# firedrakeproject/fiat

Hardware: AMD Instinct MI355X
Metric: element tabulations/sec (basis+grad, fp64) for batched P3 tet (higher is better)
Workload: dtype f64; 1 GPU; Lagrange degree 3 tetrahedron, order 1, 23 points/request, batch 100000 per GPU; requests_per_gpu=100000, points_per_request=23, order=1, points=random per request, world_size=1, launch=single process, clock_ramp_steps=224

## Files before the change

fiat_amd/csrc/api.hip:

```cpp
#include <hip/hip_runtime.h>

#include <algorithm>
#include <cmath>
#include <cstdarg>
#include <cstdio>
#include <cstring>
#include <cstdlib>
#include <mutex>
#include <string>
#include <thread>
#include <numeric>
#include <vector>

#include "../../include/fiat_amd.h"
#include "aux_kernels.hpp"
#include "plan.hpp"
#include "simplex_kernel.hpp"
#include "simplex_fixed.hpp"
#include "simplex_stream.hpp"
#include "simplex_pair.hpp"
#include "coop_kernel.hpp"
#include "shared_points.hpp"
#include "quadrature.hpp"
#include "simplex_small.hpp"
// ... 1688 lines not shown
                        !(order == 0 && vec3_rows && npts >= 17 && npts <= 24) &&
                        !(verts && order != 1 && (hi14 || hi_more)) &&
                        !(want_mix && wg_mix_takes(k)))
                        continue;
                    wg_g = npts > 64 ? 1 : std::min(12, 128 / npts);
                    wg_ctw = std::max(4, (wg_g * npts + 15) / 16);
                    if (want_mix) {
                        wg_ctw = fxwg::mix_ct(k.sd, k.n, wg_ctw);
                        wg_odd = ((long long)rows * npts) % 2 || ((long long)(rows - 16 * ((rows + 15) / 16 - 1)) * npts) % 2;
                        wg_mix1 = wg_ctw > 0 && fxwg::has_mix_instance(k.sd, k.n, wg_ctw, wg_odd) && wg_mix_takes(k);
                    }
                    if (!wg_mix1) {
                        if (verts && order >= 1 && npts <= 48 && !(ctx->policy & FX_POLICY_WG_SMALL) && !(hi14 && order == 2)) continue;
                        wg_odd = !even;
                        wg_ctw = std::max(4, (wg_g * npts + 15) / 16);
                        if (wg_ctw == 7) wg_ctw = 8;
                        if (wg_ctw == 5) {
                            const long long one = (long long)((RT + 3) / 4) * 5, two = (long long)((RT + 1) / 2) * 3;
                            if (two < one || wg_g > 1) wg_ctw = 6;
                        }
                        if (npts > 64 && (wg_g * npts + 15) / 16 <= 6 && !(ctx->policy & FX_POLICY_WG_SMALL) &&
                            !((e->nexp + 3) / 4 >= 14 || (k.sd == 2 && k.n == 6 && order == 2) || wg_ctw == 5))
                            continue;
                        if (!fxwg::has_instance(k.sd, k.n, wg_ctw, wg_odd)) continue;
                    }
                    if (!wg_mix1 && npts > 48 && npts <= 64 && even && !(ctx->policy & FX_POLICY_WG_SMALL) && !(k.sd == 3 && k.n >= 5)) {
                        bool whole = false;
                        for (const StackedShape& o : kStackedShapes)
                            whole = whole || (o.sd == k.sd && o.n == k.n && o.rtc == 0 && o.g == 1 && o.ct == 4);
                        if (whole) continue;
                    }
                    if (nreq + 3LL * ctx->num_cu > 0x7fffffffLL) continue;
                } else if (chunked) {
                    if (npts < 13 || nreq * (long long)((npts + 16 * k.ct - 1) / (16 * k.ct)) > 0x7fffffffLL) continue;
                    if ((k.rtc == -1 || k.rtc == -4) && k.sd == 3 && (k.n == 6 || k.n == 5)) {
                        const long long t2 = 2LL * ((npts + 31) / 32), t3 = 3LL * ((npts + 47) / 48);
                        if ((k.ct == 2) != (t2 < t3)) continue;
                    }
                    if (inmix) {
                        const bool nomix = (ctx->policy & FX_POLICY_NO_STACKED_MIX) != 0;
                        if (nomix || !verts || order != (k.rtc == -4 ? 1 : 2) || npts <= 16 * k.ct) continue;
                        if (k.rtc == -4 && wg_mix_takes(k)) continue;
                        if (npts <= 64 && even && R <= 224 && !(order == 2 && k.sd == 2 && k.n == 6)) {
                            bool whole = false;
                            for (const StackedShape& o : kStackedShapes)
                                whole = whole || (o.sd == k.sd && o.n == k.n && o.rtc == 0 && o.g == 1 && o.ct == 4);
                            if (whole) continue;
                        }
                    }
                } else {
                    const bool odd_twin = (k.sd == 3 && k.n == 4 && k.ct == 3 && k.g == 2) || (k.sd == 3 && k.n == 2 && k.ct == 3 && (k.g == 2 || k.g == 4)) ||
                                          (k.sd == 3 && k.n == 3 && k.ct == 3 && k.g == 2) || (k.sd == 2 && k.n == 5 && k.ct == 2 && k.g == 1);
                    if (!even && !odd_twin) continue;
                    if (npts > 16 * k.ct / k.g || tighter_instance(k) || !fills_tiles(k)) continue;
                }
                bool ok = false;
                if (e->sd == 3 && e->n == 6) ok = table_matches<3, 6>(e->prog);
                if (e->sd == 3 && e->n == 5) ok = table_matches<3, 5>(e->prog);
                if (e->sd == 3 && e->n == 4) ok = table_matches<3, 4>(e->prog);
                if (e->sd == 3 && e->n == 3) ok = table_matches<3, 3>(e->prog);
                if (e->sd == 2 && e->n == 6) ok = table_matches<2, 6>(e->prog);
                if (e->sd == 2 && e->n == 5) ok = table_matches<2, 5>(e->prog);
                if (e->sd == 3 && e->n == 2) ok = table_matches<3, 2>(e->prog);
                if (e->sd == 2 && e->n == 4) ok = table_matches<2, 4>(e->prog);
                if (e->sd == 2 && e->n == 3) ok = table_matches<2, 3>(e->prog);
                if (e->sd == 3 && e->n == 7) ok = table_matches<3, 7>(e->prog);
                if (e->sd == 2 && e->n == 7) ok = table_matches<2, 7>(e->prog);
                if (e->sd == 2 && e->n == 8) ok = table_matches<2, 8>(e->prog);
                if (!ok) continue;
                int rc = ensure_stacked(ctx, const_cast<fx_element*>(e), order);
                if (rc != FX_OK) return rc;
                if (e->stack_state[order] != 1) continue;
                fxk::StackedArgs<0>& ka = L.khead;
                memset(&ka, 0, sizeof ka);
                L.fcoef.resize(e->prog.steps.size() * 3);
                for (size_t q = 0; q < e->prog.steps.size(); ++q) {
                    L.fcoef[3 * q + 0] = e->prog.steps[q].A;
                    L.fcoef[3 * q + 1] = e->prog.steps[q].B;
                    L.fcoef[3 * q + 2] = e->prog.steps[q].C;
                }
                ka.pts = pts;
                ka.verts = verts;
                ka.out = out;
                const bool dofmajor = inmix || wg_mix1;
                ka.afrag = pio ? e->d_astack_dmp[order] : dofmajor ? e->d_astack_dm[order] : e->d_astack[order];
                if (!ka.afrag) continue;
                if (pio) {
                    for (int q = 0; q < 9; ++q) ka.G[q] = 0.5 * e->A0[q];
                    ka.piola = mapping;
                }
                if (dofmajor && !invert_small(e->sd, e->A0, ka.A0inv)) continue;
                ka.phi0 = e->prog.phi0;
                memcpy(ka.A0, e->A0, sizeof ka.A0);
                memcpy(ka.b0, e->b0, sizeof ka.b0);
                ka.nreq = nreq;
                ka.npts = npts;
                ka.R = (int)R;
                ka.RT = RT;
                ka.debug = a.debug;
                ka.lim_pts = (long long)nreq * npts * e->sd;
                ka.lim_verts = verts ? (long long)nreq * (e->sd + 1) * e->sd : 0;
                ka.lim_out = (long long)nreq * R * npts;
                const int TRk = fxk::stacked_tile_rows(e->sd, pio ? 1 : 0);
                ka.lim_afrag = (dofmajor ? ((long long)((rows + TRk - 1) / TRk) * ntab + 1) : (long long)(RT + 1)) * ((e->nexp + 3) / 4) * 64;
                const bool mixr = pio || k.rtc == -3 || k.rtc == -4 || k.rtc == -5 || (k.rtc == -2 && (mix_odd || mixr1(k.sd, k.n, k.ct, k.g) || (k.sd == 3 && k.n == 6 && k.ct == 3)));
                const int slots = fxk::stacked_mix_slots(e->sd, dofmajor ? ntab : 0, mixr);
                L.klds_bytes = (fxk::WQ_CTL_DOUBLES + STACKED_NW * (fxk::stacked_image_doubles(k.ct, (e->nexp + 3) / 4, slots) + (mixr ? fxk::STACKED_KBUF : 0))) * 8;
                if (wgk) {
                    L.klds_bytes = fxwg::lds_bytes(k.sd, k.n, wg_ctw);
                    L.wg_ct = wg_ctw;
                    L.wg_mix = wg_mix1 ? 1 : 0;
                    ka.gslab = wg_g;
                }
                if (L.klds_bytes > ctx->lds_per_cu) continue;
                const long long groups = wgk ? ((nreq + wg_g - 1) / wg_g) * STACKED_NW : chunked ? nreq * ((npts + 16 * k.ct - 1) / (16 * k.ct)) : (nreq + k.g - 1) / k.g;
                const int wgs = wgk ? fxwg::workgroups_per_cu(k.sd, k.n, wg_ctw, wg_odd, wg_mix1 ? 1 : 0, RT) : 1;
                L.kgrid = (int)std::max<long long>(1, std::min<long long>((groups + STACKED_NW - 1) / STACKED_NW, (long long)ctx->num_cu * wgs));
                L.ncu = ctx->num_cu;
                L.trash = ctx->d_trash;
                L.ctx = ctx;
                L.kmix_order = order;
                L.kodd = wgk ? wg_odd : ((k.rtc == 0 && !even) || mix_odd);
                L.kpiola = pio ? mapping : 0;
                if (pio) L.fused_mapping = true;
                L.stacked_id = (int)i;
                L.small_id = -1;
                if (fixed_yields) L.fixed_id = -1;
                break;
            }
        }
    }
    int per_cu = std::max(1, std::min(16, ctx->lds_per_cu / std::max(1, L.lds_bytes)));
    long long want = (long long)ctx->num_cu * per_cu * 4;
    L.grid = (int)std::max<long long>(1, std::min<long long>(a.nitems, want));
    return FX_OK;
}

int run_tabulate(fx_ctx* ctx, const fx_element* e, int order, const Launch& L, hipStream_t s) {
    if (L.args.nitems == 0 || L.args.npts == 0) return FX_OK;
    if (L.fixed_id >= 0) return run_fixed(L, s);
    if (L.stacked_id >= 0) return run_stacked(L, s);
    if (L.coop_id >= 0) return run_coop(L, s);
    if (L.small_id >= 0) return run_small(order, L, s);
    switch (e->sd) {
        case 1: return launch_sd<1>(order, L, s);
        case 2: return launch_sd<2>(order, L, s);
        case 3: return launch_sd<3>(order, L, s);
    }
    return fail(FX_EINVAL, "Invalid number of spatial dimensions");
}

}

namespace {
template <int SD, int ORDER, bool PIOLA, int EL>
bool launch_shared_reg_sliced(int units, const fxk::SharedArgs& sa_in, int ncu, hipStream_t s) {
    constexpr int NTAB = fxk::NTab<SD, ORDER>::value;
    constexpr int PER = EL * NTAB * (PIOLA ? SD : 1);
    constexpr int NPMAX = PER >= 80 ? 1 : PER >= 40 ? 2 : PER >= 27 ? 3 : 4;
    const int need = (units + 255) / 256;
    const int np = std::min(need, NPMAX);
    const int slices = (need + np - 1) / np;
    fxk::SharedArgs sa = sa_in;
    const long long want = 4LL * ncu;
    sa.rb = (int)std::max<long long>(1, std::min<long long>(fxk::SHARED_RB, sa.nreq * slices / want));
    const long long blocks = (sa.nreq + sa.rb - 1) / sa.rb;
    const dim3 g((unsigned)std::max<long long>(1, std::min<long long>(blocks, std::max<long long>(1, 8LL * ncu / slices))), (unsigned)slices);
    switch (np) {
        case 1: hipLaunchKernelGGL((fxk::shared_points_reg_kernel<SD, ORDER, 1, PIOLA, EL>), g, dim3(256), 0, s, sa); return true;
        case 2: if constexpr (NPMAX >= 2) { hipLaunchKernelGGL((fxk::shared_points_reg_kernel<SD, ORDER, 2, PIOLA, EL>), g, dim3(256), 0, s, sa); return true; } break;
        case 3: if constexpr (NPMAX >= 3) { hipLaunchKernelGGL((fxk::shared_points_reg_kernel<SD, ORDER, 3, PIOLA, EL>), g, dim3(256), 0, s, sa); return true; } break;
        case 4: if constexpr (NPMAX >= 4) { hipLaunchKernelGGL((fxk::shared_points_reg_kernel<SD, ORDER, 4, PIOLA, EL>), g, dim3(256), 0, s, sa); return true; } break;
    }
    return false;
}

#ifndef FX_SHARED_FLAT_MAX
#define FX_SHARED_FLAT_MAX 12
#endif
static inline bool noflat_shared(unsigned policy) { return (policy & FX_POLICY_NO_SHARED_REG) != 0 && (policy & FX_POLICY_NO_SHARED_WAVE) != 0; }

template <int SD>
int launch_shared(int order, const fxk::SharedArgs& sa, int ncu, hipStream_t s, unsigned policy) {
    const int table = sa.rows * sa.npts;
    const int grid = (int)std::max<long long>(1, std::min<long long>((sa.nreq + fxk::SHARED_RB - 1) / fxk::SHARED_RB, (long long)ncu * 8));
    {
        const long long total = (long long)fx::binom(SD + order, SD) * table;
        if (!noflat_shared(policy) && (total <= FX_SHARED_FLAT_MAX || ((table & 1) && total <= 32)) && (sa.kind == 0 || sa.vdim == SD)) {
            const long long teams = (sa.nreq + 63) / 64;
            const int fgrid = (int)std::max<long long>(1, std::min<long long>((teams + 3) / 4, (long long)grid));
            switch (order) {
                case 0: hipLaunchKernelGGL((fxk::shared_points_flat_kernel<SD, 0>), dim3(fgrid), dim3(256), 0, s, sa); break;
                case 1: hipLaunchKernelGGL((fxk::shared_points_flat_kernel<SD, 1>), dim3(fgrid), dim3(256), 0, s, sa); break;
                default: hipLaunchKernelGGL((fxk::shared_points_flat_kernel<SD, 2>), dim3(fgrid), dim3(256), 0, s, sa); break;
            }
            HIP_TRY(hipGetLastError());
            return FX_OK;
        }
    }
    const bool nowave = (policy & FX_POLICY_NO_SHARED_WAVE) != 0;
    if (!nowave && sa.kind == 0 && order == 1 && (table & 1) == 0) {
        const int npairs = (1 + SD) * table / 2;
        const int ns = (npairs + 63) / 64;
        const int nwr = ns <= 8 ? 1 : ns <= 16 ? 2 : 4;
        const long long teams = (sa.nreq + 63) / 64;
        const int wgrid = (int)std::max<long long>(1, std::min<long long>((teams * nwr + 3) / 4, (long long)grid));
        bool ok = ns <= 32;
        if (ok) hipLaunchKernelGGL((fxk::shared_points_wave_kernel<SD, 8>), dim3(wgrid), dim3(256), 0, s, sa, nwr);
        if (ok) {
            HIP_TRY(hipGetLastError());
            return FX_OK;
        }
    }
    const bool noreg = (policy & FX_POLICY_NO_SHARED_REG) != 0;
    if (!noreg && (sa.kind == 0 || sa.vdim == SD)) {
        const bool piola = sa.kind != 0;
        bool ok = false;
        constexpr bool PIO_EVEN = SD >= 2, PIO_ODD = SD == 3;
        if (table & 1) {
            if (!piola) {
                if (order == 0) ok = launch_shared_reg_sliced<SD, 0, false, 1>(table, sa, ncu, s);
                if (order == 1) ok = launch_shared_reg_sliced<SD, 1, false, 1>(table, sa, ncu, s);
                if (order == 2) ok = launch_shared_reg_sliced<SD, 2, false, 1>(table, sa, ncu, s);
            } else if constexpr (PIO_ODD) {
                if (order == 0) ok = launch_shared_reg_sliced<SD, 0, true, 1>(table, sa, ncu, s);
                if (order == 1) ok = launch_shared_reg_sliced<SD, 1, true, 1>(table, sa, ncu, s);
                if (order == 2) ok = launch_shared_reg_sliced<SD, 2, true, 1>(table, sa, ncu, s);
            }
        } else {
            if (!piola) {
                if (order == 0) ok = launch_shared_reg_sliced<SD, 0, false, 2>(table / 2, sa, ncu, s);
                if (order == 1) ok = launch_shared_reg_sliced<SD, 1, false, 2>(table / 2, sa, ncu, s);
                if (order == 2) ok = launch_shared_reg_sliced<SD, 2, false, 2>(table / 2, sa, ncu, s);
            } else if constexpr (PIO_EVEN) {
                if (order == 0) ok = launch_shared_reg_sliced<SD, 0, true, 2>(table / 2, sa, ncu, s);
                if (order == 1) ok = launch_shared_reg_sliced<SD, 1, true, 2>(table / 2, sa, ncu, s);
                if (order == 2) ok = launch_shared_reg_sliced<SD, 2, true, 2>(table / 2, sa, ncu, s);
            }
        }
        if (ok) {
            HIP_TRY(hipGetLastError());
            return FX_OK;
        }
    }
    const int rgrid = (int)std::max<long long>(1, std::min<long long>(sa.nreq, (long long)ncu * 8));
    switch (order) {
        case 0: hipLaunchKernelGGL((fxk::shared_points_kernel<SD, 0>), dim3(rgrid), dim3(256), 0, s, sa); break;
        case 1: hipLaunchKernelGGL((fxk::shared_points_kernel<SD, 1>), dim3(rgrid), dim3(256), 0, s, sa); break;
        default: hipLaunchKernelGGL((fxk::shared_points_kernel<SD, 2>), dim3(rgrid), dim3(256), 0, s, sa); break;
    }
    HIP_TRY(hipGetLastError());
    return FX_OK;
}
}

namespace {
template <int N, int NN, int ORDER>
void launch_prism_small(const fxk::PrismArgs& a, int grid, size_t lds, hipStream_t s) {
    auto kern = fxk::prism_small_kernel<N, NN, ORDER, 4>;
    if (lds > 48 * 1024) (void)hipFuncSetAttribute(reinterpret_cast<const void*>(kern), hipFuncAttributeMaxDynamicSharedMemorySize, (int)lds);
    hipLaunchKernelGGL(kern, dim3(grid), dim3(256), lds, s, a);
}
template <int N, int NN>
bool launch_prism_small_order(int order, const fxk::PrismArgs& a, int grid, size_t lds, hipStream_t s) {
    if (order == 0) launch_prism_small<N, NN, 0>(a, grid, lds, s);
    else if (order == 1) launch_prism_small<N, NN, 1>(a, grid, lds, s);
    else if (order == 2 && N <= 2 && NN <= 3) {
        if constexpr (N <= 2 && NN <= 3) launch_prism_small<N, NN, 2>(a, grid, lds, s);
    } else return false;
    return true;
}
template <int N>
bool launch_prism_small_nn(int nn, int order, const fxk::PrismArgs& a, int grid, size_t lds, hipStream_t s) {
    switch (nn) {
        case 1: return launch_prism_small_order<N, 1>(order, a, grid, lds, s);
        case 2: return launch_prism_small_order<N, 2>(order, a, grid, lds, s);
        case 3: return launch_prism_small_order<N, 3>(order, a, grid, lds, s);
        case 4: return launch_prism_small_order<N, 4>(order, a, grid, lds, s);
    }
    return false;
}
}

namespace {
template <int NF, int NN, int ORDER>
static void launch_tensor_small(bool grid_mode, const fxk::TensorArgs& a, int P, int img_doubles, int grid, size_t lds, hipStream_t s) {
    if (grid_mode) {
        auto kern = fxk::tensor_small_kernel<NF, NN, ORDER, true>;
        if (lds > 48 * 1024) (void)hipFuncSetAttribute(reinterpret_cast<const void*>(kern), hipFuncAttributeMaxDynamicSharedMemorySize, (int)lds);
        hipLaunchKernelGGL(kern, dim3(grid), dim3(256), lds, s, a, P, img_doubles);
    } else {
        auto kern = fxk::tensor_small_kernel<NF, NN, ORDER, false>;
        if (lds > 48 * 1024) (void)hipFuncSetAttribute(reinterpret_cast<const void*>(kern), hipFuncAttributeMaxDynamicSharedMemorySize, (int)lds);
        hipLaunchKernelGGL(kern, dim3(grid), dim3(256), lds, s, a, P, img_doubles);
    }
}

static bool try_tensor_small(fx_ctx* ctx, bool grid_mode, const fxk::TensorArgs& a, hipStream_t s) {
    if ((ctx->policy & FX_POLICY_NO_SMALL) != 0 || a.nf < 2 || a.npts > 64) return false;
    const int nn = a.L[0].nn;
    for (int f = 1; f < a.nf; ++f)
        if (a.L[f].nn != nn) return false;
    long long ndof = 1;
    for (int f = 0; f < a.nf; ++f) ndof *= nn;
    const long long total = (long long)a.ntab * ndof * a.npts;
    constexpr long long IMG_BYTES = 16 * 1024;
    if (total * 8 > IMG_BYTES) return false;
    const int P = (int)std::max<long long>(1, std::min<long long>(64 / a.npts, IMG_BYTES / (total * 8)));
    const int img_doubles = (int)((P * total + 1) & ~1LL);
    const size_t lds = (size_t)img_doubles * 8 * 4;
    const long long items = (a.nreq + P - 1) / P;
    const int per_cu = (int)std::max<size_t>(1, std::min<size_t>(4, (size_t)ctx->lds_per_cu / std::max<size_t>(lds, 1)));
    const int grid = (int)std::max<long long>(1, std::min<long long>((items + 3) / 4, (long long)ctx->num_cu * per_cu * 2));
    const int key = a.nf * 100 + nn * 10 + a.order;
    switch (key) {
        case 220: launch_tensor_small<2, 2, 0>(grid_mode, a, P, img_doubles, grid, lds, s); return true;
        case 221: launch_tensor_small<2, 2, 1>(grid_mode, a, P, img_doubles, grid, lds, s); return true;
        case 222: launch_tensor_small<2, 2, 2>(grid_mode, a, P, img_doubles, grid, lds, s); return true;
        case 230: launch_tensor_small<2, 3, 0>(grid_mode, a, P, img_doubles, grid, lds, s); return true;
        case 231: launch_tensor_small<2, 3, 1>(grid_mode, a, P, img_doubles, grid, lds, s); return true;
        case 232: launch_tensor_small<2, 3, 2>(grid_mode, a, P, img_doubles, grid, lds, s); return true;
        case 240: launch_tensor_small<2, 4, 0>(grid_mode, a, P, img_doubles, grid, lds, s); return true;
        case 241: launch_tensor_small<2, 4, 1>(grid_mode, a, P, img_doubles, grid, lds, s); return true;
        case 242: launch_tensor_small<2, 4, 2>(grid_mode, a, P, img_doubles, grid, lds, s); return true;
        case 250: launch_tensor_small<2, 5, 0>(grid_mode, a, P, img_doubles, grid, lds, s); return true;
        case 251: launch_tensor_small<2, 5, 1>(grid_mode, a, P, img_doubles, grid, lds, s); return true;
        case 320: launch_tensor_small<3, 2, 0>(grid_mode, a, P, img_doubles, grid, lds, s); return true;
        case 321: launch_tensor_small<3, 2, 1>(grid_mode, a, P, img_doubles, grid, lds, s); return true;
        case 322: launch_tensor_small<3, 2, 2>(grid_mode, a, P, img_doubles, grid, lds, s); return true;
        case 330: launch_tensor_small<3, 3, 0>(grid_mode, a, P, img_doubles, grid, lds, s); return true;
    }
    return false;
}

}

extern "C" {

int fx_tabulate_batch(fx_ctx* ctx, const fx_element* e, int order, int64_t nreq, int npts, const double* pts,
                      const double* verts, double* out, void* stream) {
    if (ctx && e && order > 2) {
        if (order > FX_MAX_ORDER) return fail(FX_ENOTIMPL, "derivative order %d > %d is not implemented on the device", order, FX_MAX_ORDER);
        if (nreq < 0 || npts < 0) return fail(FX_EINVAL, "negative batch size");
        if (nreq == 0 || npts == 0) return FX_OK;
        int rc = ensure_high_order(ctx, const_cast<fx_element*>(e), order);
        if (rc != FX_OK) return rc;
        rc = fx_tabulate_batch(ctx, e->high[order], 0, nreq, npts, pts, verts, out, stream);
        if (rc != FX_OK || !verts) return rc;
        return mix_high_order(ctx, e, order, nreq, npts, verts, out, (hipStream_t)stream);
    }
    Launch L;
    int rc = plan_launch(ctx, e, order, nreq, npts, pts, verts, out, L);
    if (rc != FX_OK) return rc;
    return run_tabulate(ctx, e, order, L, (hipStream_t)stream);
}

int fx_tabulate_batch_mapped(fx_ctx* ctx, const fx_element* e, int mapping, int order, int64_t nreq, int npts,
                             const double* pts, const double* verts, double* out, void* stream) {
    if (mapping < FX_MAP_AFFINE || mapping > FX_MAP_COVARIANT_CONTRAVARIANT_PIOLA) return fail(FX_EINVAL, "unknown mapping %d", mapping);
    if (mapping == FX_MAP_AFFINE) return fx_tabulate_batch(ctx, e, order, nreq, npts, pts, verts, out, stream);
    if (!e) return fail(FX_EINVAL, "null context/element");
// ... 1577 lines not shown
```

fiat_amd/csrc/shared_points.hpp:

```cpp
#pragma once
#include "simplex_kernel.hpp"
#include "store.hpp"

namespace fxk {

struct SharedArgs {
    const double* ref;
    const double* verts;
    double* out;
    double A0inv[9];
    long long nreq;
    int rows, vdim, npts, kind;
    int rb;
};

template <int SD, int ORDER> __global__ __launch_bounds__(256) void shared_points_kernel(const SharedArgs a) {
    constexpr int NTAB = NTab<SD, ORDER>::value;
    constexpr int NH = SD * (SD + 1) / 2;
    __shared__ double sK[SD * SD], sP[SD * SD], sH[NH * NH];
    const int table = a.rows * a.npts;
    const int total = NTAB * table;
    for (long long req = blockIdx.x; req < a.nreq; req += gridDim.x) {
        __syncthreads();
        if (threadIdx.x == 0) {
// ... 166 lines not shown
        }
        __builtin_amdgcn_fence(__ATOMIC_RELEASE, "wavefront", "local");
        __builtin_amdgcn_wave_barrier();
    }
}

constexpr int SHARED_RB = 64;

template <int SD, int ORDER, int NP, bool PIOLA, int EL = 2>
__global__ __launch_bounds__(256) void shared_points_reg_kernel(const SharedArgs a) {
    constexpr int NTAB = NTab<SD, ORDER>::value;
    constexpr int NH = SD * (SD + 1) / 2;
    constexpr int NE = PIOLA ? SD : 1;
    const int table = a.rows * a.npts;
    const int npairs = EL == 2 ? table >> 1 : table;
    typedef double v2d_t __attribute__((ext_vector_type(2)));
    double rv[NP][EL][NTAB][NE];
    int comp[NP][EL];
    const int pair0 = (int)blockIdx.y * NP * 256;
#pragma unroll
    for (int i = 0; i < NP; ++i) {
        const int pr = min(pair0 + (int)threadIdx.x + 256 * i, npairs - 1);
#pragma unroll
        for (int el = 0; el < EL; ++el) {
            const int q = EL * pr + el;
            const int row = q / a.npts, p = q - row * a.npts;
            comp[i][el] = PIOLA ? row % SD : 0;
            const int dof = PIOLA ? row / SD : 0;
#pragma unroll
            for (int s = 0; s < NTAB; ++s)
#pragma unroll
                for (int e = 0; e < NE; ++e)
                    rv[i][el][s][e] = PIOLA ? a.ref[(size_t)s * table + (dof * SD + e) * a.npts + p] : a.ref[(size_t)s * table + q];
        }
    }
    __shared__ double sK[SHARED_RB][SD * SD];
    const int RB = a.rb;
    for (long long base = (long long)blockIdx.x * RB; base < a.nreq; base += (long long)gridDim.x * RB) {
        __syncthreads();
        if ((int)threadIdx.x < RB) {
            const long long rq = min(base + (long long)threadIdx.x, a.nreq - 1);
            double A[SD][SD], b[SD];
            cell_map<SD>(a.verts + (size_t)rq * (SD + 1) * SD, A, b);
#pragma unroll
            for (int c = 0; c < SD; ++c)
#pragma unroll
                for (int d = 0; d < SD; ++d) {
                    double t = 0.0;
#pragma unroll
                    for (int k = 0; k < SD; ++k) t += a.A0inv[c * SD + k] * A[k][d];
                    sK[threadIdx.x][c * SD + d] = t;
                }
        }
        __syncthreads();
        const int nblk = (int)min((long long)RB, a.nreq - base);
      for (int rb = 0; rb < nblk; ++rb) {
        const long long req = base + rb;
        double K[SD][SD];
#pragma unroll
        for (int c = 0; c < SD; ++c)
#pragma unroll
            for (int d = 0; d < SD; ++d) K[c][d] = sK[rb][c * SD + d];
        double P[SD][SD];
        if constexpr (PIOLA) {
#pragma unroll
            for (int c = 0; c < SD; ++c)
#pragma unroll
                for (int e = 0; e < SD; ++e) {
                    double v;
                    if (a.kind == 1) {
                        v = K[e][c];
                    } else if constexpr (SD == 2) {
                        v = (c == e ? K[1 - c][1 - e] : -K[c][e]);
                    } else if constexpr (SD == 3) {
                        constexpr int nx[3] = {1, 2, 0}, nn[3] = {2, 0, 1};
                        v = K[nx[e]][nx[c]] * K[nn[e]][nn[c]] - K[nx[e]][nn[c]] * K[nn[e]][nx[c]];
                    } else {
                        v = 1.0;
                    }
                    P[c][e] = v;
                }
        }
        double H[NH][NH];
        if constexpr (ORDER >= 2) {
            int hd = 0;
#pragma unroll
            for (int d = 0; d < SD; ++d)
#pragma unroll
                for (int e = d; e < SD; ++e, ++hd) {
                    int hc = 0;
#pragma unroll
                    for (int c = 0; c < SD; ++c)
#pragma unroll
                        for (int c2 = c; c2 < SD; ++c2, ++hc)
                            H[hd][hc] = c == c2 ? K[c][d] * K[c][e] : K[c][d] * K[c2][e] + K[c2][d] * K[c][e];
                }
        }
        double* o1 = a.out + (size_t)req * NTAB * table;
        v2d_t* o2 = reinterpret_cast<v2d_t*>(o1);
        (void)o2;
#pragma unroll
        for (int i = 0; i < NP; ++i) {
            const int pr = pair0 + (int)threadIdx.x + 256 * i;
            if (pr < npairs) {
                double m[EL][NTAB];
#pragma unroll
                for (int el = 0; el < EL; ++el)
#pragma unroll
                    for (int s = 0; s < NTAB; ++s) {
                        if constexpr (PIOLA) {
                            double v = 0.0;
#pragma unroll
                            for (int e = 0; e < SD; ++e) {
                                double pc = P[0][e];
#pragma unroll
                                for (int c = 1; c < SD; ++c) pc = comp[i][el] == c ? P[c][e] : pc;
                                v += pc * rv[i][el][s][e];
                            }
                            m[el][s] = v;
                        } else {
                            m[el][s] = rv[i][el][s][0];
                        }
                    }
#pragma unroll
                for (int t = 0; t < NTAB; ++t) {
                    double vv[2] = {0.0, 0.0};
#pragma unroll
                    for (int el = 0; el < EL; ++el) {
                        double acc;
                        if (t == 0) {
                            acc = m[el][0];
                        } else if (t <= SD) {
                            acc = 0.0;
#pragma unroll
                            for (int c = 0; c < SD; ++c) acc += K[c][t - 1] * m[el][1 + c];
                        } else {
                            acc = 0.0;
                            if constexpr (ORDER >= 2) {
#pragma unroll
                                for (int hc = 0; hc < NH; ++hc) acc += H[t - 1 - SD][hc] * m[el][1 + SD + hc];
                            }
                        }
                        vv[el] = acc;
                    }
                    if constexpr (EL == 2) o2[(size_t)t * npairs + pr] = v2d_t{vv[0], vv[1]};
                    else o1[(size_t)t * npairs + pr] = vv[0];
                }
            }
        }
      }
    }
}

template <int SD, int NS> __global__ __launch_bounds__(256) void shared_points_wave_kernel(const SharedArgs a, const int nwr) {
    constexpr int NTAB = 1 + SD;
    const int table = a.rows * a.npts;
    const int npairs = (NTAB * table) >> 1;
    const int lane = threadIdx.x & 63;
    const int wave = __builtin_amdgcn_readfirstlane((int)(threadIdx.x >> 6));
    const int part = wave % nwr;
    const int team = (blockIdx.x * 4 + wave) / nwr;
    const long long nteams = (long long)gridDim.x * 4 / nwr;
    typedef double v2d_t __attribute__((ext_vector_type(2)));
    double rv[NS][2][SD];
    int tsel[NS];
#pragma unroll
    for (int i = 0; i < NS; ++i) {
        const int f0 = 64 * (NS * part + i);
        const int f = min(f0 + lane, npairs - 1);
        const int t = (2 * f) / table, q = 2 * f - t * table;
        tsel[i] = t;
#pragma unroll
        for (int el = 0; el < 2; ++el)
#pragma unroll
            for (int c = 0; c < SD; ++c) rv[i][el][c] = t == 0 ? (c == 0 ? a.ref[q + el] : 0.0) : a.ref[(size_t)(1 + c) * table + q + el];
    }
    __shared__ double sK[4][64][SD * SD];
    for (long long base = (long long)team * 64; base < a.nreq; base += nteams * 64) {
        {
            const long long rq = min(base + lane, a.nreq - 1);
            double A[SD][SD], b[SD];
            cell_map<SD>(a.verts + (size_t)rq * (SD + 1) * SD, A, b);
#pragma unroll
            for (int c = 0; c < SD; ++c)
#pragma unroll
                for (int d = 0; d < SD; ++d) {
                    double t = 0.0;
#pragma unroll
                    for (int k = 0; k < SD; ++k) t += a.A0inv[c * SD + k] * A[k][d];
                    sK[wave][lane][c * SD + d] = t;
                }
        }
        __builtin_amdgcn_fence(__ATOMIC_RELEASE, "wavefront", "local");
        __builtin_amdgcn_wave_barrier();
        __builtin_amdgcn_fence(__ATOMIC_ACQUIRE, "wavefront", "local");
        const int nblk = (int)min(64LL, a.nreq - base);
        for (int rb = 0; rb < nblk; ++rb) {
            double K[SD][SD];
#pragma unroll
            for (int c = 0; c < SD; ++c)
#pragma unroll
                for (int d = 0; d < SD; ++d) K[c][d] = sK[wave][rb][c * SD + d];
            v2d_t* o2 = reinterpret_cast<v2d_t*>(a.out + (size_t)(base + rb) * NTAB * table);
#pragma unroll
            for (int i = 0; i < NS; ++i) {
                const int f = 64 * (NS * part + i) + lane;
                double w[SD];
#pragma unroll
                for (int c = 0; c < SD; ++c) {
                    double x = c == 0 ? 1.0 : 0.0;
#pragma unroll
                    for (int d = 0; d < SD; ++d) x = tsel[i] == 1 + d ? K[c][d] : x;
                    w[c] = x;
                }
                v2d_t v;
                double acc0 = 0.0, acc1 = 0.0;
#pragma unroll
                for (int c = 0; c < SD; ++c) {
                    acc0 += w[c] * rv[i][0][c];
                    acc1 += w[c] * rv[i][1][c];
                }
                v.x = acc0;
                v.y = acc1;
                if (f < npairs) o2[f] = v;
            }
        }
        __builtin_amdgcn_fence(__ATOMIC_RELEASE, "wavefront", "local");
        __builtin_amdgcn_wave_barrier();
    }
}

}
```

Baseline: 380.9 million tabulations/s.

## Add dense flattened-output path to shared-points wave kernel with LDS reference tables

Adds a dense mode to the shared-points wave kernel for order-1 tables with at least 64 output pairs. The reference tables are staged once per workgroup in LDS. Output is tiled into flat 64-pair pieces spread across all waves in a persistent grid of a few workgroups per CU. Each lane prefetches the vertices of the next piece's cells while the current batch is being written, then rebuilds the Jacobians in LDS, and stores use nontemporal writes. This is meant to remove padding waste and imbalance from per-request team mapping and to keep stores contiguous. In exchange it adds per-piece integer division and modulo work, extra LDS use, and a low occupancy default that relies on the software prefetch to hide latency.

```diff
diff --git a/fiat_amd/csrc/api.hip b/fiat_amd/csrc/api.hip
--- a/fiat_amd/csrc/api.hip
+++ b/fiat_amd/csrc/api.hip
@@ -1864,6 +1864,9 @@
 
 }
 
+#ifndef FX_SHARED_REG_WG_PER_CU
+#define FX_SHARED_REG_WG_PER_CU 8
+#endif
 namespace {
 template <int SD, int ORDER, bool PIOLA, int EL>
 bool launch_shared_reg_sliced(int units, const fxk::SharedArgs& sa_in, int ncu, hipStream_t s) {
@@ -1877,7 +1880,7 @@
     const long long want = 4LL * ncu;
     sa.rb = (int)std::max<long long>(1, std::min<long long>(fxk::SHARED_RB, sa.nreq * slices / want));
     const long long blocks = (sa.nreq + sa.rb - 1) / sa.rb;
-    const dim3 g((unsigned)std::max<long long>(1, std::min<long long>(blocks, std::max<long long>(1, 8LL * ncu / slices))), (unsigned)slices);
+    const dim3 g((unsigned)std::max<long long>(1, std::min<long long>(blocks, std::max<long long>(1, (long long)FX_SHARED_REG_WG_PER_CU * ncu / slices))), (unsigned)slices);
     switch (np) {
         case 1: hipLaunchKernelGGL((fxk::shared_points_reg_kernel<SD, ORDER, 1, PIOLA, EL>), g, dim3(256), 0, s, sa); return true;
         case 2: if constexpr (NPMAX >= 2) { hipLaunchKernelGGL((fxk::shared_points_reg_kernel<SD, ORDER, 2, PIOLA, EL>), g, dim3(256), 0, s, sa); return true; } break;
@@ -1889,6 +1892,9 @@
 
 #ifndef FX_SHARED_FLAT_MAX
 #define FX_SHARED_FLAT_MAX 12
+#endif
+#ifndef FX_SHARED_DENSE_WG_PER_CU
+#define FX_SHARED_DENSE_WG_PER_CU 1
 #endif
 static inline bool noflat_shared(unsigned policy) { return (policy & FX_POLICY_NO_SHARED_REG) != 0 && (policy & FX_POLICY_NO_SHARED_WAVE) != 0; }
 
@@ -1916,9 +1922,15 @@
         const int ns = (npairs + 63) / 64;
         const int nwr = ns <= 8 ? 1 : ns <= 16 ? 2 : 4;
         const long long teams = (sa.nreq + 63) / 64;
-        const int wgrid = (int)std::max<long long>(1, std::min<long long>((teams * nwr + 3) / 4, (long long)grid));
+        int wgrid = (int)std::max<long long>(1, std::min<long long>((teams * nwr + 3) / 4, (long long)grid));
+        const int dense = npairs >= 64 ? 1 : 0;
+        static_assert(32 * 64 == fxk::SHARED_DENSE_MAX_PAIRS, "the LDS copy of the reference tables holds ns <= 32 slots");
+        if (dense) {
+            const long long npieces = (sa.nreq * (long long)npairs + 63) / 64;
+            wgrid = (int)std::max<long long>(1, std::min<long long>((npieces + 3) / 4, (long long)ncu * FX_SHARED_DENSE_WG_PER_CU));
+        }
         bool ok = ns <= 32;
-        if (ok) hipLaunchKernelGGL((fxk::shared_points_wave_kernel<SD, 8>), dim3(wgrid), dim3(256), 0, s, sa, nwr);
+        if (ok) hipLaunchKernelGGL((fxk::shared_points_wave_kernel<SD, 8>), dim3(wgrid), dim3(256), 0, s, sa, nwr, dense);
         if (ok) {
             HIP_TRY(hipGetLastError());
             return FX_OK;
diff --git a/fiat_amd/csrc/shared_points.hpp b/fiat_amd/csrc/shared_points.hpp
--- a/fiat_amd/csrc/shared_points.hpp
+++ b/fiat_amd/csrc/shared_points.hpp
@@ -342,16 +342,135 @@
     }
 }
 
-template <int SD, int NS> __global__ __launch_bounds__(256) void shared_points_wave_kernel(const SharedArgs a, const int nwr) {
+#ifndef FX_SHARED_DENSE_NT
+#define FX_SHARED_DENSE_NT 1
+#endif
+#ifndef FX_SHARED_DENSE_LATE
+#define FX_SHARED_DENSE_LATE 16
+#endif
+constexpr int SHARED_DENSE_MAX_PAIRS = 2048;
+
+template <int SD, int NS> __global__ __launch_bounds__(256) void shared_points_wave_kernel(const SharedArgs a, const int nwr, const int dense) {
     constexpr int NTAB = 1 + SD;
     const int table = a.rows * a.npts;
     const int npairs = (NTAB * table) >> 1;
     const int lane = threadIdx.x & 63;
     const int wave = __builtin_amdgcn_readfirstlane((int)(threadIdx.x >> 6));
+    typedef double v2d_t __attribute__((ext_vector_type(2)));
+    __shared__ double sK[4][129][SD * SD];
+    if (dense) {
+        __shared__ v2d_t sref[SHARED_DENSE_MAX_PAIRS + 1];
+        {
+            double* sref1 = reinterpret_cast<double*>(sref);
+            for (int i = threadIdx.x; i < NTAB * table; i += 256) sref1[i] = a.ref[i];
+            if (threadIdx.x < 2) sref1[2 * SHARED_DENSE_MAX_PAIRS + threadIdx.x] = 0.0;
+            if (lane < SD * SD) sK[wave][128][lane] = lane == 0 ? 1.0 : 0.0;
+        }
+        __syncthreads();
+        const int half = table >> 1;
+        const long long total = a.nreq * (long long)npairs;
+        const long long npieces = (total + 63) >> 6;
+        const long long W = (long long)gridDim.x * 4;
+        const int dr = (int)((unsigned)(64 * W) % (unsigned)npairs);
+        v2d_t* const o2 = reinterpret_cast<v2d_t*>(a.out);
+        const double* const sK0 = &sK[wave][0][0];
+        constexpr int NV = (SD + 1) * SD;
+        auto fetch = [&](const long long pb, double (&V)[2][NV], int& pos) {
+            const long long pi = min(pb + (long long)lane * W, npieces - 1);
+            const unsigned long long f = (unsigned long long)pi << 6;
+            const unsigned long long r = f / (unsigned long long)npairs;
+            pos = (int)(f - r * (unsigned long long)npairs);
+#pragma unroll
+            for (int h = 0; h < 2; ++h) {
+                const double* v = a.verts + (size_t)min((long long)r + h, a.nreq - 1) * NV;
+#pragma unroll
+                for (int i = 0; i < NV; ++i) V[h][i] = v[i];
+            }
+        };
+        auto build = [&](const double (&V)[2][NV]) {
+#pragma unroll
+            for (int h = 0; h < 2; ++h) {
+                double A[SD][SD], b[SD];
+                cell_map<SD>(V[h], A, b);
+#pragma unroll
+                for (int c = 0; c < SD; ++c)
+#pragma unroll
+                    for (int d = 0; d < SD; ++d) {
+                        double t = 0.0;
+#pragma unroll
+                        for (int k = 0; k < SD; ++k) t += a.A0inv[c * SD + k] * A[k][d];
+                        sK[wave][2 * lane + h][d * SD + c] = t;
+                    }
+            }
+            __builtin_amdgcn_fence(__ATOMIC_RELEASE, "wavefront", "local");
+            __builtin_amdgcn_wave_barrier();
+            __builtin_amdgcn_fence(__ATOMIC_ACQUIRE, "wavefront", "local");
+        };
+        double V[2][NV];
+        int posl;
+        long long p0 = (long long)blockIdx.x * 4 + wave;
+        if (p0 < npieces) {
+            fetch(p0, V, posl);
+            build(V);
+        }
+        for (; p0 < npieces; p0 += 64 * W) {
+            int pos0 = __builtin_amdgcn_readfirstlane(posl);
+            auto piece = [&](const int k, const bool guarded) {
+                int pos = pos0 + lane;
+                const bool second = pos >= npairs;
+                pos -= second ? npairs : 0;
+                int t = pos >= half ? 1 : 0;
+                if constexpr (SD >= 2) t += pos >= 2 * half ? 1 : 0;
+                if constexpr (SD >= 3) t += pos >= 3 * half ? 1 : 0;
+                const int value = t == 0 ? -1 : 0;
+                const int kcol = (2 * k + (second ? 1 : 0)) * SD * SD + (t - 1) * SD;
+                const double* wv = sK0 + ((kcol & ~value) | (128 * SD * SD & value));
+                const int g0 = pos + (1 - t) * half;
+                double acc0 = 0.0, acc1 = 0.0;
+#pragma unroll
+                for (int c = 0; c < SD; ++c) {
+                    const v2d_t g = sref[t == 0 ? (c == 0 ? pos : SHARED_DENSE_MAX_PAIRS) : g0 + c * half];
+                    const double w = wv[c];
+                    acc0 += w * g.x;
+                    acc1 += w * g.y;
+                }
+                v2d_t v;
+                v.x = acc0;
+                v.y = acc1;
+                const long long f = ((p0 + (long long)k * W) << 6) + lane;
+                if (!guarded || f < total) {
+#if FX_SHARED_DENSE_NT
+                    __builtin_nontemporal_store(v, &o2[f]);
+#else
+                    o2[f] = v;
+#endif
+                }
+                pos0 += dr;
+                pos0 -= pos0 >= npairs ? npairs : 0;
+            };
+            const long long pn = p0 + 64 * W;
+            if (pn < npieces) {
+#pragma unroll 4
+                for (int k = 0; k < 64 - FX_SHARED_DENSE_LATE; ++k) piece(k, false);
+                fetch(pn, V, posl);
+#pragma unroll
+                for (int k = 64 - FX_SHARED_DENSE_LATE; k < 64; ++k) piece(k, false);
+                __builtin_amdgcn_fence(__ATOMIC_RELEASE, "wavefront", "local");
+                __builtin_amdgcn_wave_barrier();
+                __builtin_amdgcn_sched_barrier(0);
+                build(V);
+            } else {
+                const int nk = (int)min(64LL, (npieces - p0 + W - 1) / W);
+#pragma unroll 4
+                for (int k = 0; k < nk - 1; ++k) piece(k, false);
+                piece(nk - 1, true);
+            }
+        }
+        return;
+    }
     const int part = wave % nwr;
     const int team = (blockIdx.x * 4 + wave) / nwr;
     const long long nteams = (long long)gridDim.x * 4 / nwr;
-    typedef double v2d_t __attribute__((ext_vector_type(2)));
     double rv[NS][2][SD];
     int tsel[NS];
 #pragma unroll
@@ -365,7 +484,6 @@
 #pragma unroll
             for (int c = 0; c < SD; ++c) rv[i][el][c] = t == 0 ? (c == 0 ? a.ref[q + el] : 0.0) : a.ref[(size_t)(1 + c) * table + q + el];
     }
-    __shared__ double sK[4][64][SD * SD];
     for (long long base = (long long)team * 64; base < a.nreq; base += nteams * 64) {
         {
             const long long rq = min(base + lane, a.nreq - 1);
```

New measurement: 374.3 million tabulations/s. -1.7%, worse.
